# vlongle/pixie

Hardware: AMD Instinct MI355X
Metric: voxels/s (128^3 U-Net fwd) + MPM particle-steps/s (higher is better)
Workload: dtype f32 (operands split fp16 hi+lo, 3 f16 MFMAs/product, fp32 accumulate); 1 GPU; 128^3x64 feature grid -> SegmentationUNet+RegressionUNet forward (+argmax/one-hot combine), 1 scene per GPU per step; grid=128, feature_channels=64, parallelism=scene-parallel x1, executor=c+hip_graph

## Files before the change

### pixie_amd/csrc/conv16_body.h

```cpp
#pragma once
#include <type_traits>

#include "conv16_device.h"

namespace pixie {

template <int KS, int MB, int NB, bool EX = false, bool SP = false, int SK = 0, bool PAIR = false>
__device__ __forceinline__ void conv3d_f16x3_body(const Conv16Args& A) {
    static_assert(!PAIR || (MB == 2 && !EX && !SP && SK == 0), "pair form: the plain f16x3 body with 64 c_out per quartet");
    static_assert(!SP || (KS == 3 && NB == 4 && !EX), "sub-pixel path: 3^3, two x parities x two voxel blocks per wave");
    static_assert(SK == 0 || (!EX && !SP), "folded skip (SK: 1 register-fed, 2 staged through LDS): f16x3, no sub-pixel form");
    extern __shared__ uint4 smem16[];
    constexpr int PAD = (KS == 3) ? 1 : 0;
    constexpr int NW = 4, NT = 64 * NW;
    const int bufsz = 4 * A.CS;

    const int tid = threadIdx.x;
    const int lane = tid & 63;
    const int quartet = PAIR ? __builtin_amdgcn_readfirstlane(tid >> 8) : 0;
    const int wave = PAIR ? (tid >> 6) & 3 : tid >> 6;
    const int qtid = PAIR ? tid & 255 : tid;
    const int kh = lane >> 5;
    const int l31 = lane & 31;

    int t = blockIdx.x;
    {
        const int per = (A.n_tiles + 7) >> 3;
        const int cand = (t & 7) * per + (t >> 3);
        if ((A.n_tiles & 7) == 0) t = cand;
    }
    int par = 0;
    if constexpr (SP) { par = t & 3; t >>= 2; }
    const int py = par & 1, pz = par >> 1;
    const int tx = t % A.tiles_x; t /= A.tiles_x;
    const int ty = t % A.tiles_y;
    const int tz = t / A.tiles_y;
    const int ox0 = tx * A.TX, oy0 = ty * A.TY, oz0 = tz * A.TZ;
    const int cout0 = (PAIR ? 2 * (int)blockIdx.y + quartet : (int)blockIdx.y) * (MB * 32);
    const int lx0 = SP ? ox0 - 1 : ox0 * A.stride - PAD;
    const int ly0 = SP ? oy0 - 1 + py : oy0 * A.stride - PAD;
    const int lz0 = SP ? oz0 - 1 + pz : oz0 * A.stride - PAD;
    const size_t ISP = (size_t)A.ID * A.IH * A.IW;
    const size_t OSP = (size_t)A.OD * A.OH * A.OW;

    int voff[NB];
    int ovox[NB];
    bool valid[NB];
#pragma unroll
    for (int nb = 0; nb < NB; ++nb) {
        if constexpr (SP) {
            const int px = nb >> 1;
            const int j = (wave * 2 + (nb & 1)) * 32 + l31;
            int x = j & (A.TX - 1);
            int y = (j >> A.lTX) & (A.TY - 1);
            int z = j >> (A.lTX + A.lTY);
            const int gx = 2 * (ox0 + x) + px, gy = 2 * (oy0 + y) + py, gz = 2 * (oz0 + z) + pz;
            const bool v = (z < A.TZ) && (gx < A.OW) && (gy < A.OH) && (gz < A.OD);
            if (!v) { x = 0; y = 0; z = 0; }
            voff[nb] = (z * A.HY + y) * A.HX + x + px + kh * A.CS;
            ovox[nb] = v ? (gz * A.OH + gy) * A.OW + gx : 0;
            valid[nb] = v;
            continue;
        }
        const int j = (wave * NB + nb) * 32 + l31;
        int x = j & (A.TX - 1);
        int y = (j >> A.lTX) & (A.TY - 1);
        int z = j >> (A.lTX + A.lTY);
        const bool v = (z < A.TZ) && (ox0 + x < A.OW) && (oy0 + y < A.OH) && (oz0 + z < A.OD);
        if (!v) { x = 0; y = 0; z = 0; }
        voff[nb] = ((z * A.HY + y) * A.HX + x) * A.stride + kh * A.CS;
        ovox[nb] = ((oz0 + z) * A.OH + (oy0 + y)) * A.OW + ox0 + x;
        valid[nb] = v;
    }

    float bound = A.in_bound;
    if (A.amax0) {
        bound = __uint_as_float(*A.amax0);
        if (A.amax1) bound = fmaxf(bound, __uint_as_float(*A.amax1));
    }
    const int ex = EX ? 0 : scale_exponent(bound);
    const float sx = pow2i(ex);

    f32x16 acc[MB][NB];
#pragma unroll
    for (int mb = 0; mb < MB; ++mb)
#pragma unroll
        for (int nb = 0; nb < NB; ++nb)
#pragma unroll
            for (int r = 0; r < 16; ++r) acc[mb][nb][r] = 0.0f;

    const int KG = A.cin >> 3;
    const size_t tap_stride = (size_t)KG * A.coutp;
    const size_t plane = (size_t)(SP ? 64 : KS * KS * KS) * tap_stride;
    const uint4* wHi = A.w16 + kW16HeaderU4 + (size_t)kh * A.coutp + cout0 + l31 + (size_t)(par * 16) * tap_stride;
    const uint4* wLo = wHi + plane;
    const float* wF = A.wf + (size_t)kh * A.coutp + cout0 + l31;

    constexpr int TAPS = KS * KS * KS;
#include "conv16_stage.h"
#include "conv16_taps.h"

    float inv2 = 0.0f;
    {
        const int c_begin = A.partial ? (int)blockIdx.z * A.chunks_per_slice * 16 : 0;
        const int c_end = A.partial ? min(A.cin, c_begin + A.chunks_per_slice * 16) : A.cin;
        if constexpr (PAIR) {
            const int n_chunks = (c_end - c_begin) >> 4;
            const int half = (A.CS + 1) >> 1;
            const int s0 = quartet ? half : 0, s1 = quartet ? A.CS : half;
#pragma unroll 1
            for (int h = -1; h < 2 * n_chunks; ++h) {
                const int k = h >> 1;
                const bool stage = (h < 0 || ((h + quartet) & 1) == 0) && k + 1 < n_chunks;
                const bool multiply = h >= 0 && ((h + quartet) & 1) != 0;
                if (stage) stage_chunk(c_begin + 16 * (k + 1), smem16 + ((k + 1) & 1) * bufsz, qtid, NT, s0, s1);
                if (multiply) mfma_chunk(c_begin + 16 * k, smem16 + (k & 1) * bufsz);
                if (h & 1) __syncthreads();
            }
        } else {
            for (int c_base = c_begin; c_base < c_end; c_base += 16) {
                __syncthreads();
                stage_chunk(c_base, smem16, tid, NT, 0, A.CS);
                __syncthreads();
                mfma_chunk(c_base, smem16);
            }
        }
#include "conv16_skip.h"
    }

#include "conv16_epilogue.h"
}

template <int KS, int MB, int NB>
__global__ __launch_bounds__(256, 2) void conv3d_f16x3_kernel(Conv16Args A) {
    conv3d_f16x3_body<KS, MB, NB>(A);
}
template <int KS, int NB>
__global__ __launch_bounds__(512, 1) void conv3d_f16x3_pair_kernel(Conv16Args A) {
    conv3d_f16x3_body<KS, 2, NB, false, false, 0, true>(A);
}
template <int KS, int MB, int NB, bool STAGED>
__global__ __launch_bounds__(256, 2) void conv3d_f16x3_skip_kernel(Conv16Args A) {
    conv3d_f16x3_body<KS, MB, NB, false, false, STAGED ? 2 : 1>(A);
}
template <int KS, int MB, int NB>
__global__ __launch_bounds__(256, 2) void conv3d_exact_kernel(Conv16Args A) {
    conv3d_f16x3_body<KS, MB, NB, true>(A);
}
template <int MB>
__global__ __launch_bounds__(256, 2) void conv3d_f16x3_subpixel_kernel(Conv16Args A) {
    conv3d_f16x3_body<3, MB, 4, false, true>(A);
}
__global__ __launch_bounds__(256, 2) void conv3d_f16x3_c64_fullres_kernel(Conv16Args A) {
    conv3d_f16x3_body<3, 2, 4>(A);
}

}
```

### pixie_amd/csrc/conv16_device.h

```cpp
#pragma once
#include <hip/hip_runtime.h>

namespace pixie {

typedef float f32x16 __attribute__((ext_vector_type(16)));
typedef _Float16 f16x8 __attribute__((ext_vector_type(8)));

constexpr int kW16HeaderU4 = 4;

struct Conv16Args {
    const float* in0; const float* in1;
    int c0, cin;
    int ID, IH, IW;
    int LD, LH, LW;
    int ups;
    int stride;
    int OD, OH, OW;
    const float* pro_a; const float* pro_b; const float* gamma; const float* beta;
    int act;
    const uint4* w16;
    const float* wf;
    const float* bias;
    int cout, coutp;
    const float* residual; float* out;
    const unsigned* amax0; const unsigned* amax1;
    float in_bound;
    int TX, TY, TZ, lTX, lTY;
    int tiles_x, tiles_y, tiles_z, n_tiles;
    int HX, HY, HZ, HYX, CS;
    unsigned mHX, mHYX;
    float* stats; unsigned* out_amax;
    float* partial; int chunks_per_slice;
    int epi_lds;
    const float* sk_in0; const float* sk_in1;
    int sk_c0, sk_cin;
    const uint4* sk_w16; const float* sk_bias;
    const unsigned* sk_amax0; const unsigned* sk_amax1;
};
// ... 25 lines not shown
```

### pixie_amd/csrc/conv16_epilogue.h

```cpp
    const float inv = EX ? 1.0f : (SK != 0 ? inv2 : __uint_as_float(A.w16[0].x) * pow2i(-ex));
    if (A.partial) {
        float* dst = A.partial + (size_t)blockIdx.z * A.cout * OSP;
#pragma unroll
        for (int mb = 0; mb < MB; ++mb)
#pragma unroll
            for (int r = 0; r < 16; ++r) {
                const int co = cout0 + mb * 32 + (r & 3) + 8 * (r >> 2) + 4 * kh;
                if (co < A.cout) {
#pragma unroll
                    for (int nb = 0; nb < NB; ++nb)
                        if (valid[nb]) dst[(size_t)co * OSP + ovox[nb]] = acc[mb][nb][r] * inv;
                }
            }
        return;
    }
    constexpr int LDO_ = NB * 32 + 4;
    float* red = reinterpret_cast<float*>(smem16) + (PAIR ? (A.epi_lds ? 2 * NW * 32 * LDO_ : 0) + quartet * (NW * MB * 64) : 0);
    float wmax = 0.0f;
    const bool full = SP ? (A.epi_lds && cout0 + MB * 32 <= A.cout && (A.TX & 1) == 0 && (A.OW & 3) == 0 && NW * 64 <= A.TX * A.TY * A.TZ &&
                            2 * (ox0 + A.TX) <= A.OW && 2 * (oy0 + A.TY) <= A.OH && 2 * (oz0 + A.TZ) <= A.OD)
                         : (A.epi_lds && cout0 + MB * 32 <= A.cout && (A.TX & 3) == 0 && (A.OW & 3) == 0 && NW * NB * 32 <= A.TX * A.TY * A.TZ &&
                            ox0 + A.TX <= A.OW && oy0 + A.TY <= A.OH && oz0 + A.TZ <= A.OD);
    if (full) {
        constexpr int LDO = NB * 32 + 4;
        float* ldsO = reinterpret_cast<float*>(smem16) + (quartet * NW + wave) * (32 * LDO);
        if constexpr (!PAIR) red = reinterpret_cast<float*>(smem16) + NW * 32 * LDO;
        constexpr int LPR = NB * 8;
        constexpr int RPI = 32 / LPR;
        constexpr int NIT = 16 / RPI;
        constexpr int G = 4;
        constexpr int GPB = NIT / G;
        constexpr int NGRP = MB * GPB;
        const int rsub = l31 / LPR, colq = 4 * (l31 % LPR), nbq = colq >> 5;
        const float* nobias = EX ? A.wf : reinterpret_cast<const float*>(A.w16);
        const bool hb0 = A.bias != nullptr, hb1 = A.sk_bias != nullptr;
        float braw[MB][2];
#pragma unroll
        for (int mb = 0; mb < MB; ++mb) {
            braw[mb][0] = (hb0 ? A.bias : nobias)[cout0 + mb * 32 + l31];
            braw[mb][1] = (hb1 ? A.sk_bias : nobias)[cout0 + mb * 32 + l31];
        }
        __syncthreads();
        const int jq = SP ? wave * 64 + (colq >> 1) : (wave * NB + nbq) * 32 + (colq & 31);
        const int xq = jq & (A.TX - 1), yq = (jq >> A.lTX) & (A.TY - 1), zq = jq >> (A.lTX + A.lTY);
        const size_t ovq = SP ? ((size_t)(2 * (oz0 + zq) + pz) * A.OH + (2 * (oy0 + yq) + py)) * A.OW + 2 * (ox0 + xq)
                              : ((size_t)(oz0 + zq) * A.OH + (oy0 + yq)) * A.OW + ox0 + xq;
        const size_t orow0 = (size_t)(cout0 + kh * RPI + rsub) * OSP + ovq;
        auto rows = [&](auto res_c, auto stats_c) {
            constexpr bool RES = decltype(res_c)::value, STATS = decltype(stats_c)::value;
            size_t step = (size_t)(2 * RPI) * OSP;
            asm volatile("" : "+s"(step));
            const float* pr = A.residual + orow0;
            float* po = A.out + orow0;
            float4 r4[2][G];
            auto fetch = [&](int q) {
#pragma unroll
                for (int g = 0; g < G; ++g) { r4[q & 1][g] = *reinterpret_cast<const float4*>(pr); pr += step; }
            };
#pragma unroll
            for (int q = 0; q < NGRP; ++q) {
                const int mb = q / GPB, it0 = (q % GPB) * G;
                asm volatile("" ::: "memory");
                if (q % GPB == 0) {
                    const int brow = __float_as_int((hb0 ? braw[mb][0] : 0.0f) + (hb1 ? braw[mb][1] : 0.0f));
#pragma unroll
                    for (int r = 0; r < 16; ++r) {
                        const int row = (r & 3) + 8 * (r >> 2);
                        const int blo = __builtin_amdgcn_readlane(brow, row), bhi = __builtin_amdgcn_readlane(brow, row + 4);
                        const float bv = __int_as_float(kh ? bhi : blo);
#pragma unroll
                        for (int nb = 0; nb < NB; ++nb)
                            ldsO[((r & 3) + 8 * (r >> 2) + 4 * kh) * LDO + (SP ? 2 * ((nb & 1) * 32 + l31) + (nb >> 1) : nb * 32 + l31)] =
                                __builtin_fmaf(acc[mb][nb][r], inv, bv);
                    }
                }
                if constexpr (RES) {
                    if (q == 0) fetch(0);
                    if (q + 1 < NGRP) fetch(q + 1);
                }
                float4 v4[G];
#pragma unroll
                for (int g = 0; g < G; ++g) {
                    const int rowl = (2 * (it0 + g) + kh) * RPI + rsub;
                    v4[g] = *reinterpret_cast<const float4*>(ldsO + rowl * LDO + colq);
                    if constexpr (RES) { v4[g].x += r4[q & 1][g].x; v4[g].y += r4[q & 1][g].y; v4[g].z += r4[q & 1][g].z; v4[g].w += r4[q & 1][g].w; }
                    *reinterpret_cast<float4*>(po) = v4[g]; po += step;
                }
                if constexpr (STATS) {
                    float s1[G], s2[G];
#pragma unroll
                    for (int g = 0; g < G; ++g) {
                        const float4 v = v4[g];
                        s1[g] = (v.x + v.y) + (v.z + v.w);
                        s2[g] = (v.x * v.x + v.y * v.y) + (v.z * v.z + v.w * v.w);
                        wmax = fmaxf(fmaxf(wmax, fmaxf(fabsf(v.x), fabsf(v.y))), fmaxf(fabsf(v.z), fabsf(v.w)));
                    }
                    asm volatile("" : "+v"(wmax));
#pragma unroll
                    for (int off = LPR / 2; off > 0; off >>= 1) {
                        float t1[G], t2[G];
#pragma unroll
                        for (int g = 0; g < G; ++g) { t1[g] = __shfl_xor(s1[g], off, 64); t2[g] = __shfl_xor(s2[g], off, 64); }
#pragma unroll
                        for (int g = 0; g < G; ++g) { s1[g] += t1[g]; s2[g] += t2[g]; }
                    }
                    if ((l31 % LPR) == 0) {
#pragma unroll
                        for (int g = 0; g < G; ++g) {
                            const int rowl = (2 * (it0 + g) + kh) * RPI + rsub;
                            red[(wave * MB * 32 + mb * 32 + rowl) * 2] = s1[g]; red[(wave * MB * 32 + mb * 32 + rowl) * 2 + 1] = s2[g];
                        }
                    }
                }
            }
        };
        using T = std::true_type; using F = std::false_type;
        if (A.residual) { if (A.stats) rows(T{}, T{}); else rows(T{}, F{}); }
        else { if (A.stats) rows(F{}, T{}); else rows(F{}, F{}); }
    } else {
        if (PAIR || A.stats) __syncthreads();
#pragma unroll
        for (int mb = 0; mb < MB; ++mb) {
#pragma unroll
            for (int r = 0; r < 16; ++r) {
                const int row = mb * 32 + (r & 3) + 8 * (r >> 2) + 4 * kh;
                const int co = cout0 + row;
                float s1 = 0.0f, s2 = 0.0f;
                if (co < A.cout) {
                    const float bv = (A.bias ? A.bias[co] : 0.0f) + (A.sk_bias ? A.sk_bias[co] : 0.0f);
#pragma unroll
                    for (int nb = 0; nb < NB; ++nb) {
                        if (valid[nb]) {
                            const size_t o = (size_t)co * OSP + ovox[nb];
                            float val = acc[mb][nb][r] * inv + bv;
                            if (A.residual) val += A.residual[o];
                            A.out[o] = val;
                            s1 += val; s2 += val * val; wmax = fmaxf(wmax, fabsf(val));
                        }
                    }
                }
                if (A.stats) {
#pragma unroll
                    for (int off = 16; off > 0; off >>= 1) { s1 += __shfl_xor(s1, off, 64); s2 += __shfl_xor(s2, off, 64); }
                    if (l31 == 0) { red[(wave * MB * 32 + row) * 2] = s1; red[(wave * MB * 32 + row) * 2 + 1] = s2; }
                }
            }
        }
    }
    if (A.stats) {
        __syncthreads();
        if (qtid < MB * 32 * 2) {
            float t = red[qtid];
#pragma unroll
            for (int w = 1; w < NW; ++w) t += red[w * MB * 64 + qtid];
            A.stats[((size_t)blockIdx.x * A.coutp + cout0) * 2 + qtid] = t;
        }
        if (A.out_amax) {
#pragma unroll
            for (int off = 32; off > 0; off >>= 1) wmax = fmaxf(wmax, __shfl_xor(wmax, off, 64));
            if (lane == 0 && wmax > 0.0f) atomicMax(A.out_amax, __float_as_uint(wmax));
        }
    }
```

### pixie_amd/csrc/conv16_stage.h

```cpp
    auto stage_chunk = [&](int c_base, uint4* buf, int stid, int nthr, int s0, int s1) {
        uint4* bHi = buf;
        uint4* bLo = buf + 2 * A.CS;
        float pa[16], pb[16];
        {
            float pv = 0.0f;
            if (A.pro_a) pv = (lane & 16) ? A.pro_b[c_base + (lane & 15)] : A.pro_a[c_base + (lane & 15)];
#pragma unroll
            for (int j = 0; j < 16; ++j) {
                pa[j] = __int_as_float(__builtin_amdgcn_readlane(__float_as_int(pv), j));
                pb[j] = __int_as_float(__builtin_amdgcn_readlane(__float_as_int(pv), 16 + j));
            }
        }
        const bool has_aff = A.gamma != nullptr;
        using T = std::true_type; using F = std::false_type;
        if constexpr (EX) {
            float* bF = reinterpret_cast<float*>(buf);
            for (int v0 = stid; v0 < A.CS; v0 += 2 * nthr) {
                float val[2][16];
                float gm[2], bt[2];
                int sidx[2];
                bool ok[2];
#pragma unroll
                for (int u = 0; u < 2; ++u) {
                    const int vox = v0 + u * nthr;
// ... 79 lines not shown
            if constexpr (BUF) {
                const int voff = 4 * sidx;
                it.gm = __uint_as_float(__builtin_amdgcn_raw_buffer_load_b32(rsg, voff, 0, 0));
                it.bt = __uint_as_float(__builtin_amdgcn_raw_buffer_load_b32(rsb, voff, 0, 0));
#pragma unroll
                for (int j = 0; j < 16; ++j)
                    it.val[j] = __uint_as_float(__builtin_amdgcn_raw_buffer_load_b32(rs, voff, (int)((unsigned)j * chb), 0));
            } else {
                load_with_pointers(it, sidx);
            }
            __builtin_amdgcn_sched_barrier(0);
        };
        auto convert = [&](const Item& it, int vox, auto has_pro, auto act_c) {
            const float gm = has_aff ? it.gm : 1.0f, bt = has_aff ? it.bt : 0.0f;
            f16x8 vh[2], vl[2];
#pragma unroll
            for (int j = 0; j < 16; ++j) {
                float t = it.val[j];
                if (decltype(has_pro)::value) t = t * pa[j] + pb[j];
                t = t * gm + bt;
                const float sc = act16_staged(t, decltype(act_c)::value) * sx;
                const _Float16 h = (_Float16)sc;
                vh[j >> 3][j & 7] = h;
                vl[j >> 3][j & 7] = (_Float16)(sc - (float)h);
            }
            uint4 w[4] = {__builtin_bit_cast(uint4, vh[0]), __builtin_bit_cast(uint4, vh[1]), __builtin_bit_cast(uint4, vl[0]),
                          __builtin_bit_cast(uint4, vl[1])};
#pragma unroll
            for (int q = 0; q < 4; ++q) {
                w[q].x = it.ok ? w[q].x : 0u; w[q].y = it.ok ? w[q].y : 0u;
                w[q].z = it.ok ? w[q].z : 0u; w[q].w = it.ok ? w[q].w : 0u;
            }
            if (vox < s1) {
                bHi[vox] = w[0];
                bHi[A.CS + vox] = w[1];
                bLo[vox] = w[2];
                bLo[A.CS + vox] = w[3];
            }
            __builtin_amdgcn_sched_barrier(0);
        };
        auto pipeline = [&](auto has_pro, auto act_c) {
            Item a, b;
            int vox = s0 + stid;
            int left = n_items;
            if constexpr (BUF) {
                if (straddle) {
#pragma unroll 1
                    for (; left > 0; --left, vox += nthr) {
                        load_with_pointers(a, slot(vox, a.ok));
                        convert(a, vox, has_pro, act_c);
                    }
                    return;
                }
            }
            fetch(a, vox);
#pragma unroll 1
            for (; left > 2; left -= 2, vox += 2 * nthr) {
                fetch(b, vox + nthr);
                convert(a, vox, has_pro, act_c);
                fetch(a, vox + 2 * nthr);
                convert(b, vox + nthr, has_pro, act_c);
            }
            if (left == 2) {
                fetch(b, vox + nthr);
                convert(a, vox, has_pro, act_c);
                convert(b, vox + nthr, has_pro, act_c);
            } else {
                convert(a, vox, has_pro, act_c);
            }
        };
// ... 11 lines not shown
```

### pixie_amd/csrc/conv16_taps.h

```cpp
    auto mfma_chunk = [&](int c_base, const uint4* buf) {
        __builtin_amdgcn_s_setprio(3);
        if constexpr (EX) {
            const float* ldsF = reinterpret_cast<const float*>(buf);
            const size_t tapw = (size_t)A.cin * A.coutp;
            const float* wc = wF + (size_t)c_base * A.coutp;
            float a[8][MB], an[8][MB];
#pragma unroll
            for (int kp = 0; kp < 8; ++kp)
#pragma unroll
                for (int mb = 0; mb < MB; ++mb) a[kp][mb] = wc[(size_t)(2 * kp) * A.coutp + mb * 32];
#pragma unroll 1
            for (int zy = 0; zy < KS * KS; ++zy) {
                const int dz = zy / KS, dy = zy - dz * KS;
                const int rowoff = (dz * A.HY + dy) * A.HX;
#pragma unroll
                for (int dx = 0; dx < KS; ++dx) {
                    const int tap = zy * KS + dx;
                    const int nxt = (tap + 1 < TAPS) ? tap + 1 : tap;
#pragma unroll
                    for (int kp = 0; kp < 8; ++kp)
#pragma unroll
                        for (int mb = 0; mb < MB; ++mb) an[kp][mb] = wc[(size_t)nxt * tapw + (size_t)(2 * kp) * A.coutp + mb * 32];
                    __builtin_amdgcn_sched_barrier(0);
#pragma unroll
// ... 40 lines not shown
                    for (int mb = 0; mb < MB; ++mb) {
                        ahn[mb] = __builtin_bit_cast(f16x8, wh[nxt + mb * 32]);
                        aln[mb] = __builtin_bit_cast(f16x8, wl[nxt + mb * 32]);
                    }
                    __builtin_amdgcn_sched_barrier(0);
                    f16x8 bh[2], bl[2];
#pragma unroll
                    for (int s = 0; s < 2; ++s) {
                        bh[s] = __builtin_bit_cast(f16x8, ldsHi[voff[px * 2 + s] + rowoff + ex]);
                        bl[s] = __builtin_bit_cast(f16x8, ldsLo[voff[px * 2 + s] + rowoff + ex]);
                    }
#pragma unroll
                    for (int mb = 0; mb < MB; ++mb)
#pragma unroll
                        for (int s = 0; s < 2; ++s)
                            acc[mb][px * 2 + s] = __builtin_amdgcn_mfma_f32_32x32x16_f16(al[mb], bh[s], acc[mb][px * 2 + s], 0, 0, 0);
#pragma unroll
                    for (int mb = 0; mb < MB; ++mb)
#pragma unroll
                        for (int s = 0; s < 2; ++s)
                            acc[mb][px * 2 + s] = __builtin_amdgcn_mfma_f32_32x32x16_f16(ah[mb], bl[s], acc[mb][px * 2 + s], 0, 0, 0);
#pragma unroll
                    for (int mb = 0; mb < MB; ++mb)
#pragma unroll
                        for (int s = 0; s < 2; ++s)
                            acc[mb][px * 2 + s] = __builtin_amdgcn_mfma_f32_32x32x16_f16(ah[mb], bh[s], acc[mb][px * 2 + s], 0, 0, 0);
#pragma unroll
                    for (int mb = 0; mb < MB; ++mb) { ah[mb] = ahn[mb]; al[mb] = aln[mb]; }
                }
            }
            __builtin_amdgcn_s_setprio(0);
            return;
        }
        f16x8 ah[MB], al[MB];
#pragma unroll
        for (int mb = 0; mb < MB; ++mb) {
            ah[mb] = __builtin_bit_cast(f16x8, wh[mb * 32]);
            al[mb] = __builtin_bit_cast(f16x8, wl[mb * 32]);
        }
#pragma unroll 1
        for (int zy = 0; zy < KS * KS; ++zy) {
            const int dz = zy / KS, dy = zy - dz * KS;
            const int rowoff = (dz * A.HY + dy) * A.HX;
#pragma unroll
            for (int dx = 0; dx < KS; ++dx) {
                const int tap = zy * KS + dx;
                const int nxt = (tap + 1 < TAPS) ? tap + 1 : tap;
                f16x8 ahn[MB], aln[MB];
#pragma unroll
                for (int mb = 0; mb < MB; ++mb) {
                    ahn[mb] = __builtin_bit_cast(f16x8, wh[(size_t)nxt * tap_stride + mb * 32]);
                    aln[mb] = __builtin_bit_cast(f16x8, wl[(size_t)nxt * tap_stride + mb * 32]);
                }
                __builtin_amdgcn_sched_barrier(0);
                f16x8 bh[NB], bl[NB];
#pragma unroll
                for (int nb = 0; nb < NB; ++nb) {
                    bh[nb] = __builtin_bit_cast(f16x8, ldsHi[voff[nb] + rowoff + dx]);
                    bl[nb] = __builtin_bit_cast(f16x8, ldsLo[voff[nb] + rowoff + dx]);
                }
#pragma unroll
                for (int mb = 0; mb < MB; ++mb)
#pragma unroll
                    for (int nb = 0; nb < NB; ++nb)
                        acc[mb][nb] = __builtin_amdgcn_mfma_f32_32x32x16_f16(al[mb], bh[nb], acc[mb][nb], 0, 0, 0);
#pragma unroll
// ... 16 lines not shown
```

### pixie_amd/csrc/conv3d_f16x3.hip

```cpp
#include <hip/hip_runtime.h>

#include <cstdlib>

#include "../../include/pixie_hip.h"
#include "common.h"
#include "conv_plan.h"
#include "conv_launch.h"
#include "conv16_device.h"
#include "conv16_body.h"
#include "conv_stat_kernels.h"
#include "conv_pack_kernels.h"

namespace pixie {

bool conv_exact_v1() { return getenv("PIXIE_CONV_EXACT_V1") != nullptr; }

ConvShape conv_shape_of(const pixie_conv_desc* d) {
    ConvShape s;
    s.c0 = d->c0; s.c1 = d->c1; s.c_out = d->c_out;
    s.in_d = d->in_d; s.in_h = d->in_h; s.in_w = d->in_w;
    s.ksize = d->ksize; s.stride = d->stride; s.upsample = d->upsample;
    s.out_d = d->out_d; s.out_h = d->out_h; s.out_w = d->out_w;
    s.skip_c0 = d->skip_c0; s.skip_c1 = d->skip_c1;
    s.w16 = d->d_w16 != nullptr; s.subpixel = d->w16_subpixel != 0; s.workspace = d->d_workspace != nullptr; s.skip = d->d_skip_w16 != nullptr;
    s.exact_v1 = conv_exact_v1();
    return s;
}

using ConvKernel = void (*)(Conv16Args);
static ConvKernel conv16_kernel(const ConvPlan& p, bool skip = false, int skip_c0 = 0) {
    if (p.path == CONV_F16X3_SUBPIXEL) return p.MB == 2 ? conv3d_f16x3_subpixel_kernel<2> : conv3d_f16x3_subpixel_kernel<1>;
    if (p.fullres) return conv3d_f16x3_c64_fullres_kernel;
#define PX_CONV16_PICK(KS_, MB_, NB_)                                                                \
    if (p.KS == KS_ && p.MB == MB_ && p.NB == NB_)                                                   \
        return p.path == CONV_EXACT_TILED ? conv3d_exact_kernel<KS_, MB_, NB_>                       \
                                          : (!skip ? conv3d_f16x3_kernel<KS_, MB_, NB_>                                \
                                                   : ((skip_c0 & 8) ? conv3d_f16x3_skip_kernel<KS_, MB_, NB_, true> : conv3d_f16x3_skip_kernel<KS_, MB_, NB_, false>));
    PX_CONV_VARIANTS(PX_CONV16_PICK)
#undef PX_CONV16_PICK
    return nullptr;
}

#ifdef PIXIE_DIAG
static int g_conv_keep_four_wave = 0;
#endif
static size_t conv_pair_lds(const ConvPlan& p, bool skip) {
#ifdef PIXIE_DIAG
    if (g_conv_keep_four_wave) return 0;
#endif
    return conv_pair_lds_bytes(p, skip);
}
static ConvKernel conv16_pair_kernel(const ConvPlan& p) {
#define PX_CONV16_PAIR(KS_, NB_) \
    if (p.KS == KS_ && p.NB == NB_) return conv3d_f16x3_pair_kernel<KS_, NB_>;
    PX_CONV16_PAIR(3, 4) PX_CONV16_PAIR(1, 4)
#undef PX_CONV16_PAIR
    return nullptr;
}

static int launch(ConvKernel kern, const ConvPlan& p, const Conv16Args& a, hipStream_t st, size_t pair_lds = 0) {
    PX_REQUIRE(kern != nullptr, "conv: no kernel variant for ksize=%d MB=%d NB=%d", p.KS, p.MB, p.NB);
    PX_CHECK_HIP(allow_max_dynamic_lds(reinterpret_cast<const void*>(kern)));
    if (pair_lds) hipLaunchKernelGGL(kern, dim3(p.grid_x, p.grid_y / 2, 1), dim3(512), pair_lds, st, a);
    else hipLaunchKernelGGL(kern, dim3(p.grid_x, p.grid_y, p.grid_z), dim3(256), p.lds_bytes, st, a);
    PX_CHECK_HIP(hipGetLastError());
    return 0;
}

static Conv16Args conv16_args(const pixie_conv_desc* d, const ConvPlan& p) {
    Conv16Args a{};
    a.in0 = d->d_in0; a.in1 = d->d_in1; a.c0 = d->c0; a.cin = d->c0 + d->c1;
    a.ID = d->in_d; a.IH = d->in_h; a.IW = d->in_w;
    a.LD = p.LD; a.LH = p.LH; a.LW = p.LW; a.ups = p.ups; a.stride = d->stride;
    a.OD = p.OD; a.OH = p.OH; a.OW = p.OW;
    a.pro_a = d->d_pro_a; a.pro_b = d->d_pro_b; a.gamma = d->d_gamma; a.beta = d->d_beta; a.act = d->act;
    a.bias = d->d_bias; a.cout = d->c_out; a.coutp = p.coutp;
    a.residual = d->d_residual; a.out = d->d_out;
    a.TX = p.TX; a.TY = p.TY; a.TZ = p.TZ; a.lTX = p.lTX; a.lTY = p.lTY;
    a.tiles_x = p.tiles_x; a.tiles_y = p.tiles_y; a.tiles_z = p.tiles_z; a.n_tiles = p.n_tiles;
    a.HX = p.HX; a.HY = p.HY; a.HZ = p.HZ; a.HYX = p.HYX; a.CS = p.CS; a.mHX = p.mHX; a.mHYX = p.mHYX;
    a.chunks_per_slice = p.chunks_per_slice; a.epi_lds = p.epi_lds;
    return a;
}

int conv3d_f16x3_forward(const pixie_conv_desc* d, const ConvPlan& p, hipStream_t st) {
// ... 40 lines not shown
    }
    PX_CHECK_HIP(hipGetLastError());
    return 0;
}

int conv3d_exact_forward(const pixie_conv_desc* d, const ConvPlan& p, hipStream_t st) {
    PX_REQUIRE(p.refusal != CONV_BAD_LDS, "exact conv: tile needs %zu B of LDS", p.lds_bytes);
    PX_REQUIRE(p.path == CONV_EXACT_TILED, "exact conv: bad sizes");
    Conv16Args a = conv16_args(d, p);
    a.wf = d->d_w;
    a.in_bound = 1.0f;
    return launch(conv16_kernel(p), p, a, st);
}

}

using namespace pixie;

static ConvPlan plan_of(const pixie_conv_desc* d) { return d ? conv_plan(conv_shape_of(d)) : ConvPlan{}; }
static StatParts stat_parts(const ConvPlan& p, const void* stats) { return StatParts{stats, p.stats.n, p.stats.cstride, p.stats.tstride, p.stats.f64}; }

extern "C" int64_t pixie_conv_stats_floats(const pixie_conv_desc* d) { return plan_of(d).stats_floats; }

extern "C" int64_t pixie_conv_workspace_bytes(const pixie_conv_desc* d) {
    if (!d) return 0;
    ConvShape s = conv_shape_of(d);
    s.workspace = true;
    return conv_plan(s).workspace_bytes;
}

#ifdef PIXIE_DIAG
extern "C" int pixie_conv_kernel_variant(const pixie_conv_desc* d, int* slices_out) {
    if (!d) {
        const int before = g_conv_keep_four_wave;
        if (slices_out && (*slices_out == 0 || *slices_out == 1)) g_conv_keep_four_wave = *slices_out;
        return before;
    }
    const ConvPlan p = plan_of(d);
    if (slices_out) *slices_out = p.f16x3() ? p.slices : 1;
    return conv_variant_number(p);
}

extern "C" int pixie_conv_tile_geometry(const pixie_conv_desc* d, int32_t out[10]) {
    const ConvPlan p = plan_of(d);
    if (!out && d) return (int)conv_pair_lds(p, d->d_skip_w16 != nullptr);
    return out && conv_tile_geometry(p, out) ? 0 : 1;
}

extern "C" int pixie_conv_stats_layout(const pixie_conv_desc* d, int64_t out[6]) {
    const ConvPlan p = plan_of(d);
    return out && conv_stats_layout(p, out) ? 0 : 1;
}
#endif

extern "C" int pixie_conv_skip_foldable(const pixie_conv_desc* d) { return plan_of(d).skip_foldable ? 1 : 0; }

extern "C" int pixie_stats_finalize(const float* d_stats, const pixie_conv_desc* d, double* d_sums, void* stream) {
    PX_REQUIRE(d_stats && d && d_sums, "pixie_stats_finalize: null argument");
    hipLaunchKernelGGL(stats_finalize_kernel, dim3((unsigned)d->c_out), dim3(256), 0, as_stream(stream), stat_parts(plan_of(d), d_stats), d_sums);
    PX_CHECK_HIP(hipGetLastError());
    return 0;
}

extern "C" int pixie_stats_norm_finalize(const float* d_stats0, const pixie_conv_desc* desc0, double* d_sums0, const float* d_stats1,
                                         const pixie_conv_desc* desc1, double* d_sums1, int c1, int64_t spatial, int mode, int groups,
                                         double eps, const float* d_weight, const float* d_bias, float* d_a, float* d_b, void* stream) {
// ... 67 lines not shown
```

### pixie_amd/csrc/conv_plan.h

```cpp
#pragma once
#include <algorithm>
#include <cstddef>
#include <cstdint>

#include "../../include/pixie_hip.h"

namespace pixie {

#define PX_CONV_VARIANTS(X) \
    X(3, 2, 4) X(3, 2, 2) X(3, 2, 1) X(3, 1, 4) X(3, 1, 2) X(3, 1, 1) X(1, 2, 4) X(1, 2, 2) X(1, 2, 1) X(1, 1, 4) X(1, 1, 2) X(1, 1, 1)

struct ConvShape {
    int c0 = 0, c1 = 0, c_out = 0, in_d = 0, in_h = 0, in_w = 0, ksize = 0, stride = 1, upsample = 0;
    int out_d = 0, out_h = 0, out_w = 0;
    int skip_c0 = 0, skip_c1 = 0;
    bool w16 = false;
    bool subpixel = false;
    bool workspace = false;
    bool skip = false;
    bool exact_v1 = false;
};

enum ConvPath { CONV_NONE = 0, CONV_F16X3, CONV_F16X3_SUBPIXEL, CONV_EXACT_TILED, CONV_FIRST_GEN };
enum ConvRefusal { CONV_OK = 0, CONV_BAD_SHAPE, CONV_BAD_STRIDE, CONV_BAD_CHANNELS, CONV_BAD_SUBPIXEL, CONV_BAD_LDS };
// ... 107 lines not shown
    if (p.slices > 1) p.chunks_per_slice = (chunks + p.slices - 1) / p.slices;
    p.lds_bytes = (size_t)4 * p.CS * 16;
    if (p.lds_bytes > 160 * 1024) return refuse(CONV_BAD_LDS);
    const size_t epi_bytes = ((size_t)4 * 32 * (p.NB * 32 + 4) + (size_t)4 * p.MB * 32 * 2) * sizeof(float);
    if (p.slices == 1 && epi_bytes <= 80 * 1024) { p.epi_lds = 1; p.lds_bytes = std::max(p.lds_bytes, epi_bytes); }
    p.grid_x = (unsigned)p.n_tiles; p.grid_y = (unsigned)((p.coutp + p.MB * 32 - 1) / (p.MB * 32)); p.grid_z = (unsigned)p.slices;
    if (!p.f16x3()) return p;
    const long osp = (long)p.OD * p.OH * p.OW;
    if (p.slices > 1) {
        const int n = reduce_segments(osp);
        p.stats = ConvStatLayout{n, n, 1, 1};
        p.stats_floats = (int64_t)s.c_out * n * 2 * (int64_t)(sizeof(double) / sizeof(float));
        p.workspace_bytes = (int64_t)p.slices * s.c_out * osp * (int64_t)sizeof(float);
    } else {
        p.stats = ConvStatLayout{p.n_tiles, 1, p.coutp, 0};
        p.stats_floats = (int64_t)p.n_tiles * p.coutp * 2;
    }
    p.fullres = !sub && p.slices == 1 && s.ksize == 3 && p.MB == 2 && p.NB == 4 && cin == 64 && s.c_out == 64 && s.stride == 1 && !s.upsample &&
                s.c1 == 0 && !s.skip && osp >= 128L * 128 * 128;
    const int scin = s.skip_c0 + s.skip_c1;
    p.skip_foldable = !sub && s.stride == 1 && !s.upsample && scin > 0 && scin % 16 == 0 && s.skip_c0 % 8 == 0 && p.slices == 1;
    return p;
}

inline size_t conv_pair_lds_bytes(const ConvPlan& p, bool skip) {
    if (p.path != CONV_F16X3 || p.fullres || skip || p.MB != 2 || p.NB != 4 || p.slices != 1 || p.coutp % 128 != 0) return 0;
    const size_t tiles = (size_t)2 * 4 * p.CS * 16;
    const size_t red = (size_t)2 * 4 * p.MB * 32 * 2 * sizeof(float);
    const size_t epi = p.epi_lds ? (size_t)8 * 32 * (p.NB * 32 + 4) * sizeof(float) + red : red;
    const size_t lds = std::max(tiles, epi);
    return lds <= 160 * 1024 ? lds : 0;
}

inline int conv_variant_number(const ConvPlan& p) {
    if (!p.f16x3()) return 0;
    if (p.path == CONV_F16X3_SUBPIXEL) return 8300 + p.MB * 10 + p.NB;
    if (p.fullres) return 9324;
    return p.KS * 100 + p.MB * 10 + p.NB;
}
inline bool conv_tile_geometry(const ConvPlan& p, int32_t out[10]) {
    if (!p.tiled()) return false;
    const int32_t v[10] = {p.TX, p.TY, p.TZ, p.tiles_x, p.tiles_y, p.tiles_z, p.epi_lds, p.slices, p.MB, p.NB};
    for (int i = 0; i < 10; ++i) out[i] = v[i];
    return true;
}
inline bool conv_stats_layout(const ConvPlan& p, int64_t out[6]) {
    if (!p.f16x3()) return false;
    out[0] = p.stats.n; out[1] = p.stats.cstride; out[2] = p.stats.tstride; out[3] = p.stats.f64; out[4] = p.stats.f64 ? kReduceSeg : 0;
    out[5] = p.coutp;
    return true;
}

}
```

Measured before the change: 27.56 million voxels/s.

## Use 16x16x32 f16 MFMA tap loop for 3^3 f16x3 convolutions

Adds an M16 variant of the 3^3 f16x3 conv body that uses 16x16x32 MFMAs instead of the 32x32 form. Each lane group handles two taps at once, with the K dimension split across a tap pair. The LDS staging layout interleaves the two channel halves per voxel to match. The epilogue, partial-sum and stats paths get new lane-to-row mappings. The default path, the pair kernel and the full-res kernel all switch to this form, aiming for higher MFMA throughput and fewer wasted K steps, at the cost of more register pressure and a more complex layout.

```diff
diff --git a/pixie_amd/csrc/conv16_body.h b/pixie_amd/csrc/conv16_body.h
--- a/pixie_amd/csrc/conv16_body.h
+++ b/pixie_amd/csrc/conv16_body.h
@@ -5,8 +5,9 @@
 
 namespace pixie {
 
-template <int KS, int MB, int NB, bool EX = false, bool SP = false, int SK = 0, bool PAIR = false>
+template <int KS, int MB, int NB, bool EX = false, bool SP = false, int SK = 0, bool PAIR = false, bool M16 = false>
 __device__ __forceinline__ void conv3d_f16x3_body(const Conv16Args& A) {
+    static_assert(!M16 || (KS == 3 && MB == 2 && NB == 4 && !EX && !SP && SK == 0), "16x16x32 tap loop: the plain 3^3 f16x3 body, 64 c_out x 128 voxels per wave");
     static_assert(!PAIR || (MB == 2 && !EX && !SP && SK == 0), "pair form: the plain f16x3 body with 64 c_out per quartet");
     static_assert(!SP || (KS == 3 && NB == 4 && !EX), "sub-pixel path: 3^3, two x parities x two voxel blocks per wave");
     static_assert(SK == 0 || (!EX && !SP), "folded skip (SK: 1 register-fed, 2 staged through LDS): f16x3, no sub-pixel form");
@@ -16,12 +17,13 @@
     const int bufsz = 4 * A.CS;
 
     const int tid = threadIdx.x;
-    const int lane = tid & 63;
+    int lane = tid & 63;
     const int quartet = PAIR ? __builtin_amdgcn_readfirstlane(tid >> 8) : 0;
-    const int wave = PAIR ? (tid >> 6) & 3 : tid >> 6;
-    const int qtid = PAIR ? tid & 255 : tid;
-    const int kh = lane >> 5;
-    const int l31 = lane & 31;
+    int wave = PAIR ? (tid >> 6) & 3 : tid >> 6;
+    int qtid = PAIR ? tid & 255 : tid;
+    int kh = lane >> 5;
+    int l31 = lane & 31;
+    int c15 = lane & 15, kg = lane >> 4;
 
     int t = blockIdx.x;
     {
@@ -72,6 +74,27 @@
         ovox[nb] = ((oz0 + z) * A.OH + (oy0 + y)) * A.OW + ox0 + x;
         valid[nb] = v;
     }
+    auto geo16 = [&](int n, int ln, int& slot, int& ov) {
+        const int j = wave * 128 + n * 16 + (ln & 15);
+        int x = j & (A.TX - 1);
+        int y = (j >> A.lTX) & (A.TY - 1);
+        int z = j >> (A.lTX + A.lTY);
+        const bool v = (z < A.TZ) && (ox0 + x < A.OW) && (oy0 + y < A.OH) && (oz0 + z < A.OD);
+        ov = ((oz0 + z) * A.OH + (oy0 + y)) * A.OW + ox0 + x;
+        if (!v) { x = 0; y = 0; z = 0; }
+        slot = (z * A.HY + y) * A.HX + x;
+        return v;
+    };
+    unsigned voff16[M16 ? NB : 1];
+    if constexpr (M16) {
+#pragma unroll
+        for (int n = 0; n < 2 * NB; ++n) {
+            int slot, ov;
+            geo16(n, lane, slot, ov);
+            const unsigned v = (unsigned)(2 * slot + (kg & 1));
+            voff16[n >> 1] = (n & 1) ? (voff16[n >> 1] | (v << 16)) : v;
+        }
+    }
 
     float bound = A.in_bound;
     if (A.amax0) {
@@ -95,6 +118,7 @@
     const uint4* wHi = A.w16 + kW16HeaderU4 + (size_t)kh * A.coutp + cout0 + l31 + (size_t)(par * 16) * tap_stride;
     const uint4* wLo = wHi + plane;
     const float* wF = A.wf + (size_t)kh * A.coutp + cout0 + l31;
+    const uint4* wHi16 = A.w16 + kW16HeaderU4 + (size_t)(kg & 1) * A.coutp + cout0 + c15;
 
     constexpr int TAPS = KS * KS * KS;
 #include "conv16_stage.h"
@@ -128,6 +152,12 @@
 #include "conv16_skip.h"
     }
 
+    if constexpr (M16) {
+        int t2 = threadIdx.x;
+        asm volatile("" : "+v"(t2));
+        lane = t2 & 63; wave = PAIR ? (t2 >> 6) & 3 : t2 >> 6; qtid = PAIR ? t2 & 255 : t2;
+        kh = lane >> 5; l31 = lane & 31; c15 = lane & 15; kg = lane >> 4;
+    }
 #include "conv16_epilogue.h"
 }
 
@@ -151,8 +181,14 @@
 __global__ __launch_bounds__(256, 2) void conv3d_f16x3_subpixel_kernel(Conv16Args A) {
     conv3d_f16x3_body<3, MB, 4, false, true>(A);
 }
+__global__ __launch_bounds__(256, 2) void conv3d_f16x3_m16_kernel(Conv16Args A) {
+    conv3d_f16x3_body<3, 2, 4, false, false, 0, false, true>(A);
+}
+__global__ __launch_bounds__(512, 1) void conv3d_f16x3_pair_m16_kernel(Conv16Args A) {
+    conv3d_f16x3_body<3, 2, 4, false, false, 0, true, true>(A);
+}
 __global__ __launch_bounds__(256, 2) void conv3d_f16x3_c64_fullres_kernel(Conv16Args A) {
-    conv3d_f16x3_body<3, 2, 4>(A);
+    conv3d_f16x3_body<3, 2, 4, false, false, 0, false, true>(A);
 }
 
 }
diff --git a/pixie_amd/csrc/conv16_device.h b/pixie_amd/csrc/conv16_device.h
--- a/pixie_amd/csrc/conv16_device.h
+++ b/pixie_amd/csrc/conv16_device.h
@@ -4,6 +4,7 @@
 namespace pixie {
 
 typedef float f32x16 __attribute__((ext_vector_type(16)));
+typedef float f32x4 __attribute__((ext_vector_type(4)));
 typedef _Float16 f16x8 __attribute__((ext_vector_type(8)));
 
 constexpr int kW16HeaderU4 = 4;
diff --git a/pixie_amd/csrc/conv16_epilogue.h b/pixie_amd/csrc/conv16_epilogue.h
--- a/pixie_amd/csrc/conv16_epilogue.h
+++ b/pixie_amd/csrc/conv16_epilogue.h
@@ -1,6 +1,33 @@
+    int ovox16[M16 ? 2 * NB : 1];
+    bool valid16[M16 ? 2 * NB : 1];
+    auto edge_geometry16 = [&]() {
+        int ln = lane;
+        asm volatile("" : "+v"(ln));
+#pragma unroll
+        for (int n = 0; n < 2 * NB; ++n) {
+            int slot, ov;
+            valid16[n] = geo16(n, ln, slot, ov);
+            ovox16[n] = valid16[n] ? ov : 0;
+        }
+    };
     const float inv = EX ? 1.0f : (SK != 0 ? inv2 : __uint_as_float(A.w16[0].x) * pow2i(-ex));
     if (A.partial) {
         float* dst = A.partial + (size_t)blockIdx.z * A.cout * OSP;
+        if constexpr (M16) {
+            edge_geometry16();
+#pragma unroll
+            for (int mb = 0; mb < MB; ++mb)
+#pragma unroll
+                for (int rr = 0; rr < 8; ++rr) {
+                    const int co = cout0 + mb * 32 + 16 * (rr >> 2) + 4 * kg + (rr & 3);
+                    if (co < A.cout) {
+#pragma unroll
+                        for (int n = 0; n < 2 * NB; ++n)
+                            if (valid16[n]) dst[(size_t)co * OSP + ovox16[n]] = acc[mb][n >> 1][8 * (rr >> 2) + 4 * (n & 1) + (rr & 3)] * inv;
+                    }
+                }
+            return;
+        }
 #pragma unroll
         for (int mb = 0; mb < MB; ++mb)
 #pragma unroll
@@ -63,6 +90,16 @@
                 asm volatile("" ::: "memory");
                 if (q % GPB == 0) {
                     const int brow = __float_as_int((hb0 ? braw[mb][0] : 0.0f) + (hb1 ? braw[mb][1] : 0.0f));
+                    if constexpr (M16) {
+#pragma unroll
+                        for (int rr = 0; rr < 8; ++rr) {
+                            const int row = 16 * (rr >> 2) + 4 * kg + (rr & 3);
+                            const float bv = __int_as_float(__builtin_amdgcn_ds_bpermute(4 * row, brow));
+#pragma unroll
+                            for (int n = 0; n < 2 * NB; ++n)
+                                ldsO[row * LDO + n * 16 + c15] = __builtin_fmaf(acc[mb][n >> 1][8 * (rr >> 2) + 4 * (n & 1) + (rr & 3)], inv, bv);
+                        }
+                    } else {
 #pragma unroll
                     for (int r = 0; r < 16; ++r) {
                         const int row = (r & 3) + 8 * (r >> 2);
@@ -72,6 +109,7 @@
                         for (int nb = 0; nb < NB; ++nb)
                             ldsO[((r & 3) + 8 * (r >> 2) + 4 * kh) * LDO + (SP ? 2 * ((nb & 1) * 32 + l31) + (nb >> 1) : nb * 32 + l31)] =
                                 __builtin_fmaf(acc[mb][nb][r], inv, bv);
+                    }
                     }
                 }
                 if constexpr (RES) {
@@ -119,30 +157,61 @@
         else { if (A.stats) rows(F{}, T{}); else rows(F{}, F{}); }
     } else {
         if (PAIR || A.stats) __syncthreads();
-#pragma unroll
-        for (int mb = 0; mb < MB; ++mb) {
-#pragma unroll
-            for (int r = 0; r < 16; ++r) {
-                const int row = mb * 32 + (r & 3) + 8 * (r >> 2) + 4 * kh;
-                const int co = cout0 + row;
-                float s1 = 0.0f, s2 = 0.0f;
-                if (co < A.cout) {
-                    const float bv = (A.bias ? A.bias[co] : 0.0f) + (A.sk_bias ? A.sk_bias[co] : 0.0f);
-#pragma unroll
-                    for (int nb = 0; nb < NB; ++nb) {
-                        if (valid[nb]) {
-                            const size_t o = (size_t)co * OSP + ovox[nb];
-                            float val = acc[mb][nb][r] * inv + bv;
-                            if (A.residual) val += A.residual[o];
-                            A.out[o] = val;
-                            s1 += val; s2 += val * val; wmax = fmaxf(wmax, fabsf(val));
-                        }
-                    }
-                }
-                if (A.stats) {
-#pragma unroll
-                    for (int off = 16; off > 0; off >>= 1) { s1 += __shfl_xor(s1, off, 64); s2 += __shfl_xor(s2, off, 64); }
-                    if (l31 == 0) { red[(wave * MB * 32 + row) * 2] = s1; red[(wave * MB * 32 + row) * 2 + 1] = s2; }
+        if constexpr (M16) {
+            edge_geometry16();
+#pragma unroll
+            for (int mb = 0; mb < MB; ++mb) {
+#pragma unroll
+                for (int rr = 0; rr < 8; ++rr) {
+                    const int row = mb * 32 + 16 * (rr >> 2) + 4 * kg + (rr & 3);
+                    const int co = cout0 + row;
+                    float s1 = 0.0f, s2 = 0.0f;
+                    if (co < A.cout) {
+                        const float bv = (A.bias ? A.bias[co] : 0.0f) + (A.sk_bias ? A.sk_bias[co] : 0.0f);
+#pragma unroll
+                        for (int n = 0; n < 2 * NB; ++n) {
+                            if (valid16[n]) {
+                                const size_t o = (size_t)co * OSP + ovox16[n];
+                                float val = acc[mb][n >> 1][8 * (rr >> 2) + 4 * (n & 1) + (rr & 3)] * inv + bv;
+                                if (A.residual) val += A.residual[o];
+                                A.out[o] = val;
+                                s1 += val; s2 += val * val; wmax = fmaxf(wmax, fabsf(val));
+                            }
+                        }
+                    }
+                    if (A.stats) {
+#pragma unroll
+                        for (int off = 8; off > 0; off >>= 1) { s1 += __shfl_xor(s1, off, 64); s2 += __shfl_xor(s2, off, 64); }
+                        if (c15 == 0) { red[(wave * MB * 32 + row) * 2] = s1; red[(wave * MB * 32 + row) * 2 + 1] = s2; }
+                    }
+                }
+            }
+        } else {
+#pragma unroll
+            for (int mb = 0; mb < MB; ++mb) {
+#pragma unroll
+                for (int r = 0; r < 16; ++r) {
+                    const int row = mb * 32 + (r & 3) + 8 * (r >> 2) + 4 * kh;
+                    const int co = cout0 + row;
+                    float s1 = 0.0f, s2 = 0.0f;
+                    if (co < A.cout) {
+                        const float bv = (A.bias ? A.bias[co] : 0.0f) + (A.sk_bias ? A.sk_bias[co] : 0.0f);
+#pragma unroll
+                        for (int nb = 0; nb < NB; ++nb) {
+                            if (valid[nb]) {
+                                const size_t o = (size_t)co * OSP + ovox[nb];
+                                float val = acc[mb][nb][r] * inv + bv;
+                                if (A.residual) val += A.residual[o];
+                                A.out[o] = val;
+                                s1 += val; s2 += val * val; wmax = fmaxf(wmax, fabsf(val));
+                            }
+                        }
+                    }
+                    if (A.stats) {
+#pragma unroll
+                        for (int off = 16; off > 0; off >>= 1) { s1 += __shfl_xor(s1, off, 64); s2 += __shfl_xor(s2, off, 64); }
+                        if (l31 == 0) { red[(wave * MB * 32 + row) * 2] = s1; red[(wave * MB * 32 + row) * 2 + 1] = s2; }
+                    }
                 }
             }
         }
diff --git a/pixie_amd/csrc/conv16_stage.h b/pixie_amd/csrc/conv16_stage.h
--- a/pixie_amd/csrc/conv16_stage.h
+++ b/pixie_amd/csrc/conv16_stage.h
@@ -135,10 +135,17 @@
                 w[q].z = it.ok ? w[q].z : 0u; w[q].w = it.ok ? w[q].w : 0u;
             }
             if (vox < s1) {
-                bHi[vox] = w[0];
-                bHi[A.CS + vox] = w[1];
-                bLo[vox] = w[2];
-                bLo[A.CS + vox] = w[3];
+                if constexpr (M16) {
+                    bHi[2 * vox] = w[0];
+                    bHi[2 * vox + 1] = w[1];
+                    bLo[2 * vox] = w[2];
+                    bLo[2 * vox + 1] = w[3];
+                } else {
+                    bHi[vox] = w[0];
+                    bHi[A.CS + vox] = w[1];
+                    bLo[vox] = w[2];
+                    bLo[A.CS + vox] = w[3];
+                }
             }
             __builtin_amdgcn_sched_barrier(0);
         };
diff --git a/pixie_amd/csrc/conv16_taps.h b/pixie_amd/csrc/conv16_taps.h
--- a/pixie_amd/csrc/conv16_taps.h
+++ b/pixie_amd/csrc/conv16_taps.h
@@ -96,6 +96,84 @@
             __builtin_amdgcn_s_setprio(0);
             return;
         }
+        if constexpr (M16) {
+            const uint4* ldsHi = buf;
+            const uint4* ldsLo = buf + 2 * A.CS;
+            const uint4* wh16 = wHi16 + (size_t)(c_base >> 3) * A.coutp;
+            const size_t tsel_off = (kg >> 1) ? tap_stride : 0;
+            f32x4 q[4][8];
+#pragma unroll
+            for (int m = 0; m < 4; ++m)
+#pragma unroll
+                for (int n = 0; n < 8; ++n) {
+                    const int b = 4 * (2 * (m & 1) + (n & 1));
+#pragma unroll
+                    for (int i = 0; i < 4; ++i) q[m][n][i] = acc[m >> 1][n >> 1][b + i];
+                }
+            f16x8 ah[4], al[4];
+#pragma unroll
+            for (int m = 0; m < 4; ++m) {
+                ah[m] = __builtin_bit_cast(f16x8, wh16[tsel_off + m * 16]);
+                al[m] = __builtin_bit_cast(f16x8, wh16[plane + tsel_off + m * 16]);
+            }
+            auto tap_slot = [&](int t) {
+                const int dz = t / 9, r = t - 9 * dz, dy = r / 3, dx = r - 3 * dy;
+                return 2 * ((dz * A.HY + dy) * A.HX + dx);
+            };
+            constexpr bool PIN = PAIR;
+            auto bslot = [&](int n) { return (int)((voff16[n >> 1] >> (16 * (n & 1))) & 0xffffu); };
+            auto step = [&](int boff) {
+                f16x8 bh = __builtin_bit_cast(f16x8, ldsHi[bslot(0) + boff]);
+                f16x8 bl = __builtin_bit_cast(f16x8, ldsLo[bslot(0) + boff]);
+#pragma unroll
+                for (int n = 0; n < 8; ++n) {
+#pragma unroll
+                    for (int m = 0; m < 4; ++m) q[m][n] = __builtin_amdgcn_mfma_f32_16x16x32_f16(ah[m], bl, q[m][n], 0, 0, 0);
+                    if constexpr (PIN) __builtin_amdgcn_sched_barrier(0);
+                    if (n < 7) bl = __builtin_bit_cast(f16x8, ldsLo[bslot(n + 1) + boff]);
+                    if constexpr (PIN) __builtin_amdgcn_sched_barrier(0);
+#pragma unroll
+                    for (int m = 0; m < 4; ++m) q[m][n] = __builtin_amdgcn_mfma_f32_16x16x32_f16(al[m], bh, q[m][n], 0, 0, 0);
+#pragma unroll
+                    for (int m = 0; m < 4; ++m) q[m][n] = __builtin_amdgcn_mfma_f32_16x16x32_f16(ah[m], bh, q[m][n], 0, 0, 0);
+                    if constexpr (PIN) __builtin_amdgcn_sched_barrier(0);
+                    if (n < 7) bh = __builtin_bit_cast(f16x8, ldsHi[bslot(n + 1) + boff]);
+                    if constexpr (PIN) __builtin_amdgcn_sched_barrier(0);
+                }
+            };
+#pragma unroll 1
+            for (int s = 0; s < 13; ++s) {
+                const size_t nxt = (size_t)(2 * s + 2) * tap_stride + (s < 12 ? tsel_off : 0);
+                f16x8 ahn[4], aln[4];
+#pragma unroll
+                for (int m = 0; m < 4; ++m) {
+                    ahn[m] = __builtin_bit_cast(f16x8, wh16[nxt + m * 16]);
+                    aln[m] = __builtin_bit_cast(f16x8, wh16[plane + nxt + m * 16]);
+                }
+                __builtin_amdgcn_sched_barrier(0);
+                const int b0 = tap_slot(2 * s), b1 = tap_slot(2 * s + 1);
+                step((kg >> 1) ? b1 : b0);
+#pragma unroll
+                for (int m = 0; m < 4; ++m) { ah[m] = ahn[m]; al[m] = aln[m]; }
+            }
+            if (kg >> 1) {
+#pragma unroll
+                for (int m = 0; m < 4; ++m)
+#pragma unroll
+                    for (int j = 0; j < 8; ++j) { ah[m][j] = (_Float16)0.0f; al[m][j] = (_Float16)0.0f; }
+            }
+            step(tap_slot(26));
+#pragma unroll
+            for (int m = 0; m < 4; ++m)
+#pragma unroll
+                for (int n = 0; n < 8; ++n) {
+                    const int b = 4 * (2 * (m & 1) + (n & 1));
+#pragma unroll
+                    for (int i = 0; i < 4; ++i) acc[m >> 1][n >> 1][b + i] = q[m][n][i];
+                }
+            __builtin_amdgcn_s_setprio(0);
+            return;
+        }
         f16x8 ah[MB], al[MB];
 #pragma unroll
         for (int mb = 0; mb < MB; ++mb) {
diff --git a/pixie_amd/csrc/conv3d_f16x3.hip b/pixie_amd/csrc/conv3d_f16x3.hip
--- a/pixie_amd/csrc/conv3d_f16x3.hip
+++ b/pixie_amd/csrc/conv3d_f16x3.hip
@@ -28,9 +28,18 @@
 }
 
 using ConvKernel = void (*)(Conv16Args);
+#ifdef PIXIE_DIAG
+static int g_conv_keep_mfma32 = 0;
+#endif
+static bool conv_mfma16(const ConvPlan& p, bool skip) {
+#ifdef PIXIE_DIAG
+    if (g_conv_keep_mfma32) return false;
+#endif
+    return conv_mfma16_form(p, skip);
+}
 static ConvKernel conv16_kernel(const ConvPlan& p, bool skip = false, int skip_c0 = 0) {
     if (p.path == CONV_F16X3_SUBPIXEL) return p.MB == 2 ? conv3d_f16x3_subpixel_kernel<2> : conv3d_f16x3_subpixel_kernel<1>;
-    if (p.fullres) return conv3d_f16x3_c64_fullres_kernel;
+    if (conv_mfma16(p, skip)) return p.fullres ? conv3d_f16x3_c64_fullres_kernel : conv3d_f16x3_m16_kernel;
 #define PX_CONV16_PICK(KS_, MB_, NB_)                                                                \
     if (p.KS == KS_ && p.MB == MB_ && p.NB == NB_)                                                   \
         return p.path == CONV_EXACT_TILED ? conv3d_exact_kernel<KS_, MB_, NB_>                       \
@@ -51,6 +60,7 @@
     return conv_pair_lds_bytes(p, skip);
 }
 static ConvKernel conv16_pair_kernel(const ConvPlan& p) {
+    if (conv_mfma16(p, false)) return conv3d_f16x3_pair_m16_kernel;
 #define PX_CONV16_PAIR(KS_, NB_) \
     if (p.KS == KS_ && p.NB == NB_) return conv3d_f16x3_pair_kernel<KS_, NB_>;
     PX_CONV16_PAIR(3, 4) PX_CONV16_PAIR(1, 4)
@@ -157,6 +167,11 @@
 #ifdef PIXIE_DIAG
 extern "C" int pixie_conv_kernel_variant(const pixie_conv_desc* d, int* slices_out) {
     if (!d) {
+        if (slices_out && (*slices_out == 2 || *slices_out == 3)) {
+            const int before = g_conv_keep_mfma32;
+            g_conv_keep_mfma32 = *slices_out - 2;
+            return before;
+        }
         const int before = g_conv_keep_four_wave;
         if (slices_out && (*slices_out == 0 || *slices_out == 1)) g_conv_keep_four_wave = *slices_out;
         return before;
diff --git a/pixie_amd/csrc/conv_plan.h b/pixie_amd/csrc/conv_plan.h
--- a/pixie_amd/csrc/conv_plan.h
+++ b/pixie_amd/csrc/conv_plan.h
@@ -163,6 +163,10 @@
     return lds <= 160 * 1024 ? lds : 0;
 }
 
+inline bool conv_mfma16_form(const ConvPlan& p, bool skip) {
+    return p.path == CONV_F16X3 && !skip && p.KS == 3 && p.MB == 2 && p.NB == 4;
+}
+
 inline int conv_variant_number(const ConvPlan& p) {
     if (!p.f16x3()) return 0;
     if (p.path == CONV_F16X3_SUBPIXEL) return 8300 + p.MB * 10 + p.NB;
```

New measurement: 27.81 million voxels/s (median of 6 runs). About the same (+0.9%).
